# liuzm-slam/VLOAM-NOTED

Measured on AMD Instinct MI355X. Metric: scan-to-map LM iters/sec on 64-ring KITTI-shaped cloud, higher is better.
Workload: dtype fp64 pose/normal equations, fp32 points

## Files before the change

### vloam-noted_amd/csrc/cubeindex.h

```cpp
#pragma once
#include "common.h"
#include "device_math.h"

namespace loam {

constexpr uint32_t CI_EMPTY = 0xFFFFFFFFu;
constexpr uint32_t CI_KEY_MASK = (1u << 18) - 1;
constexpr int CI_LDS_MAX_T = 32768;

__host__ __device__ inline uint32_t ci_table_size(uint32_t n) {
  uint32_t t = 1;
  while (t < 2 * n) t <<= 1;
  return t;
}
__device__ inline uint32_t ci_hash(uint32_t k, uint32_t mask) {
  uint32_t h = k * 0x9E3779B1u;
  h ^= h >> 15;
  return h & mask;
}
__device__ inline int ci_corner(int c, int cen) { return (c - cen) * 50 - 25; }
__device__ inline uint32_t ci_local_key(const float4& p, const int corner[3]) {
  const int lx = (int)floorf(p.x) - corner[0], ly = (int)floorf(p.y) - corner[1], lz = (int)floorf(p.z) - corner[2];
  return (uint32_t)(lx & 63) | ((uint32_t)(ly & 63) << 6) | ((uint32_t)(lz & 63) << 12);
}

template <int nthreads>
__device__ inline uint32_t ci_block_scan(uint32_t v, uint32_t* ws, uint32_t* total) {
  constexpr int W = nthreads / 64;
  const int wid = threadIdx.x >> 6, lane = threadIdx.x & 63;
  const uint32_t inc = wave_incl_scan_u(v);
  if (lane == 63) ws[wid] = inc;
  __syncthreads();
  if (threadIdx.x == 0) {
    uint32_t acc = 0;
    for (int w = 0; w < W; ++w) {
      const uint32_t t = ws[w];
      ws[w] = acc;
      acc += t;
    }
    ws[W] = acc;
  }
  __syncthreads();
  const uint32_t r = ws[wid] + inc - v;
  *total = ws[W];
  __syncthreads();
  return r;
}

template <int nthreads, int MAXT = CI_LDS_MAX_T>
__device__ inline bool cube_index_build(const float4* pts, uint32_t n, const int corner[3], float4* cpts,
                                        uint2* ctab, uint32_t* lds, unsigned long long* prof = nullptr) {
  const int tid = threadIdx.x;
  if (n == 0) return true;
  const uint32_t T = ci_table_size(n), mask = T - 1;
  uint32_t* ws = lds + MAXT;
  bool ok = true;
  if (prof && tid == 0 && T <= (uint32_t)MAXT && n < (1u << 14)) atomicAdd(prof, 0ull - __builtin_readcyclecounter());
  if (T <= (uint32_t)MAXT && n < (1u << 14)) {
    uint32_t* lent = lds;
    for (uint32_t i = tid; i < T; i += nthreads) lent[i] = CI_EMPTY;
    __syncthreads();
    constexpr int PER = (MAXT / 2 + nthreads - 1) / nthreads;
    constexpr int CI_LOADS = PER < 8 ? PER : 8;
    uint32_t sr[PER];
#pragma unroll
    for (int k0 = 0; k0 < PER; k0 += CI_LOADS) {
      float4 p[CI_LOADS];
#pragma unroll
      for (int u = 0; u < CI_LOADS; ++u) p[u] = pts[min(tid + (uint32_t)(k0 + u) * nthreads, n - 1)];
#pragma unroll
      for (int u = 0; u < CI_LOADS; ++u)
        sr[k0 + u] = tid + (uint32_t)(k0 + u) * nthreads < n ? ci_local_key(p[u], corner) : CI_EMPTY;
    }
    const int lane = tid & 63;
    const uint64_t le = lane == 63 ? ~0ull : ((2ull << lane) - 1ull);
#pragma unroll
    for (int k = 0; k < PER; ++k) {
      const uint32_t key = sr[k];
      const uint32_t prev = (uint32_t)__shfl_up((int)key, 1, 64);
      const uint64_t heads = __ballot(lane == 0 || prev != key);
      const int head = 63 - __clzll(heads & le);
      uint32_t base = 0;
      if (key != CI_EMPTY && head == lane) {
        const uint64_t after = heads & ~le;
        const uint32_t run = (uint32_t)((after ? __ffsll((long long)after) - 1 : 64) - lane);
        uint32_t h = ci_hash(key, mask);
        while (true) {
          const uint32_t old = atomicCAS(&lent[h], CI_EMPTY, key | (run << 18));
          if (old == CI_EMPTY) break;
          if ((old & CI_KEY_MASK) == key) {
            base = atomicAdd(&lent[h], run << 18) >> 18;
            break;
          }
          h = (h + 1) & mask;
        }
        base |= h << 15;
      }
      const uint32_t hb = (uint32_t)__shfl((int)base, head, 64);
      sr[k] = key == CI_EMPTY ? CI_EMPTY : hb + (uint32_t)(lane - head);
    }
    __syncthreads();
    if (prof && tid == 0) atomicAdd(prof, __builtin_readcyclecounter());
    uint32_t sum = 0;
    for (uint32_t h = tid; h < T; h += nthreads) {
      const uint32_t e = lent[h];
      if (e != CI_EMPTY) sum += e >> 18;
    }
    uint32_t tot;
    uint32_t pre = ci_block_scan<nthreads>(sum, ws, &tot);
    for (uint32_t h = tid; h < T; h += nthreads) {
      const uint32_t e = lent[h];
      ctab[h] = make_uint2(e, pre);
      lent[h] = pre;
      if (e != CI_EMPTY) pre += e >> 18;
    }
    __syncthreads();
#pragma unroll
    for (int k0 = 0; k0 < PER; k0 += CI_LOADS) {
      float4 p[CI_LOADS];
#pragma unroll
      for (int u = 0; u < CI_LOADS; ++u) p[u] = pts[min(tid + (uint32_t)(k0 + u) * nthreads, n - 1)];
#pragma unroll
      for (int u = 0; u < CI_LOADS; ++u) {
        const uint32_t i = tid + (uint32_t)(k0 + u) * nthreads;
        if (i < n) cpts[lent[sr[k0 + u] >> 15] + (sr[k0 + u] & 0x7FFFu)] = make_float4(p[u].x, p[u].y, p[u].z, __int_as_float((int)i));
      }
    }
    __syncthreads();
    return ok;
  }
  for (uint32_t i = tid; i < T; i += nthreads) ctab[i] = make_uint2(CI_EMPTY, 0);
  __syncthreads();
  for (uint32_t i = tid; i < n; i += nthreads) {
    const uint32_t key = ci_local_key(pts[i], corner);
    uint32_t h = ci_hash(key, mask);
    while (true) {
      const uint32_t old = atomicCAS(&ctab[h].x, CI_EMPTY, key);
      if (old == CI_EMPTY || old == key) break;
      h = (h + 1) & mask;
    }
    atomicAdd(&ctab[h].y, 1u);
  }
  __syncthreads();
  uint32_t sum = 0;
  for (uint32_t h = tid; h < T; h += nthreads) {
    const uint2 e = ctab[h];
    if (e.x != CI_EMPTY) sum += e.y;
  }
  uint32_t tot;
  uint32_t pre = ci_block_scan<nthreads>(sum, ws, &tot);
  for (uint32_t h = tid; h < T; h += nthreads) {
    const uint2 e = ctab[h];
    if (e.x == CI_EMPTY) continue;
    ok &= e.y < (1u << 14);
    ctab[h] = make_uint2(e.x | (e.y << 18), pre);
    pre += e.y;
  }
  __syncthreads();
  for (uint32_t i = tid; i < n; i += nthreads) {
    const float4 p = pts[i];
// ... 29 lines not shown
```

### vloam-noted_amd/csrc/mapper.hip

```cpp
#include <algorithm>
#include <cmath>
#include <cstdlib>
#include <array>
#include <cstring>
#include <deque>
#include <memory>
#include <vector>

#include "common.h"
#include "device_math.h"
#include "cellhash.h"
#include "comm.h"
#include "cubeindex.h"
#include "device_res.h"
#include "lm.h"
#include "voxel.h"
#include "voxel_hot.h"
#include "voxel_pcl.h"
#include "mapper_dev.h"
#include "mapper_stack.h"
#include "mapper_frame.h"
#include "mapper_corr.h"
#include "mapper_lm.h"
#include "mapper_map.h"
// ... 88 lines not shown
  StackIn* sin_buf = nullptr;
  PinnedArray<StackIn> hsin;
};

struct loam_mapper {
  DevStream st;
  DevStream st2;
  int32_t held_rc = 0;
  std::string held_msg;
  loam_params P;
  bool prof = false;
  std::vector<DevEvent> ev_pool;
  std::vector<int> ev_fam;
  double fam_ms[NFAM] = {0}, fam_bytes[NFAM] = {0};
  long long fam_launches[NFAM] = {0};
  int dev = 0, B = 1;
  DevEvent ev_opt_begin, ev_opt_end;
  MapperDev D{};
  PinnedArray<StreamFrame> hf;
  std::vector<HostStream> hs;
  uint2* cube_tab[2] = {nullptr, nullptr};
  int parity = 0;
  uint32_t* tok_tmp = nullptr;
  uint32_t* d_new_off = nullptr;
  DevPool pool;
  uint32_t frame_counter = 0;
  int n_cu = 256;
  uint32_t compact_at = 0;
  int lm_G = 0;
  bool want_ipc = false;
  DevBuf<char> ipc_own;
  std::vector<void*> ipc_open;
  int knn_cs = 0;
  loam_comm* comm = nullptr;
  PinnedArray<int> q_off;
  int* d_q_off = nullptr;
  int use_graph = 0;
  hipGraphExec_t gexec[2][2] = {{nullptr, nullptr}, {nullptr, nullptr}};
  int spar = 0, last_spar = 0;
  ParitySlot slot[2];
  std::deque<FrameRec> q;
  uint64_t seq = 0, mirror_seq = 0;
  unsigned long long stack_seq = 0;
  unsigned long long* d_stk_ready = nullptr;
  PinnedArray<unsigned long long> done;
  unsigned long long* done_dev = nullptr;
// ... 280 lines not shown
  }
  TRY(alloc(D.arena, B * 2 * 2 * (size_t)D.map_cap));
  TRY(alloc(D.carena, B * 2 * 2 * (size_t)D.map_cap));
  TRY(alloc(D.ctab, B * 2 * 2 * 4 * (size_t)D.map_cap));
  TRY(alloc(h->cube_tab[0], B * 2 * NCUBE));
  TRY(alloc(h->cube_tab[1], B * 2 * NCUBE));
  TRY(alloc(D.extra_flag, B * 2 * NCUBE));
  D.knn_stride = B * 2 * (size_t)D.max_in;
  TRY(alloc(D.knn_id, 5 * D.knn_stride));
  TRY(alloc(D.r_type, B * 2 * (size_t)D.max_in));
  TRY(alloc(D.r_px, B * 2 * (size_t)D.max_in));
  TRY(alloc(D.r_py, B * 2 * (size_t)D.max_in));
  TRY(alloc(D.r_pz, B * 2 * (size_t)D.max_in));
  for (int k = 0; k < 3; ++k) {
    TRY(alloc(D.r_a[k], B * 2 * (size_t)D.max_in));
    TRY(alloc(D.r_b[k], B * 2 * (size_t)D.max_in));
  }
  TRY(alloc(D.ins_pts, B * 2 * (size_t)D.max_in));
  TRY(alloc(D.ins_tag, B * 2 * (size_t)D.max_in));
  TRY(alloc(D.ins_sorted, B * 2 * (size_t)D.max_in));
  TRY(alloc(D.ins_off, B * 2 * (size_t)(INS_SLOTS + 1)));
  TRY(alloc(D.stable_tok, B * 2 * (size_t)NCUBE));
  TRY(alloc(h->tok_tmp, B * 2 * (size_t)NCUBE));
  TRY(alloc(D.dbg, LOAM_DEBUG_COUNTERS));
  {
    const char* penv = std::getenv("LOAM_PHASE_COUNTERS");
    D.pdbg = (penv && std::atoi(penv) > 0) ? D.dbg : nullptr;
  }
  TRY(alloc(D.vx_pts, B * 2 * (size_t)D.scratch_cap));
  if (D.pcl_order) {
    const size_t ps = mp_scratch(D);
    TRY(alloc(D.pe, B * 2 * ps));
    TRY(alloc(D.pa, B * 2 * ps));
    TRY(alloc(D.pb, B * 2 * ps));
    TRY(alloc(D.ps, B * 2 * ps));
    TRY(alloc(D.pseg, B * 2 * (mp_pseg(ps) + 9)));
  }
  TRY(alloc(D.vx_idx, B * 2 * (size_t)D.scratch_cap));
  TRY(alloc(D.stk_part, B * 2 * (size_t)STACK_K_MAX));
  for (ParitySlot& S : h->slot) {
    TRY(alloc(S.stk_n_buf, B * 2));
    TRY(alloc(S.stk_err_buf, B));
    if (B <= 4) {
      TRY(S.hsin.assign_mapped(B, StackIn{}, &S.sin_buf));
    } else {
      TRY(alloc(S.sin_buf, B));
// ... 90 lines not shown
  do {                                                                                      \
    if ((h) && !(h)->q.empty() && !(h)->q.front().behind && !(h)->q.front().early_seen) { \
      LOAM_HIP(hipSetDevice((h)->dev));                                                     \
      TRY(finish_oldest(h));                                                                \
    }                                                                                       \
  } while (0)

int32_t loam_mapper_destroy(loam_mapper* h) {
  if (!h) return LOAM_ERR_ARG;
  (void)hipSetDevice(h->dev);
  while (!h->q.empty()) (void)finish_oldest(h);
  delete h;
  return LOAM_OK;
}

int32_t loam_mapper_reset(loam_mapper* h) {
  if (!h) return LOAM_ERR_ARG;
  SETTLE(h);
  LOAM_HIP(hipSetDevice(h->dev));
  LOAM_HIP(hipStreamSynchronize(h->st2));
  for (int p = 0; p < 2; ++p)
    LOAM_HIP(hipMemsetAsync(h->cube_tab[p], 0, sizeof(uint2) * h->B * 2 * NCUBE, h->st));
  LOAM_HIP(hipMemsetAsync(h->D.stable_tok, 0, sizeof(uint32_t) * h->B * 2 * NCUBE, h->st));
  LOAM_HIP(hipStreamSynchronize(h->st));
  for (int s = 0; s < h->B; ++s) {
    h->hf[s] = fresh_record();
    h->last_tail[s] = {0u, 0u};
    h->hs[s] = HostStream{};
  }
  return LOAM_OK;
}

static int32_t mapper_input_common(loam_mapper* h, int32_t s, const float* corner, int32_t nc,
                                   const float* surf, int32_t ns, const double* q_wodom,
                                   const double* t_wodom, int32_t skip, hipMemcpyKind kind) {
  TRY(check_stream(h, s));
  if (!q_wodom || !t_wodom || nc < 0 || ns < 0 || (nc > 0 && !corner) || (ns > 0 && !surf)) {
    set_error("loam_mapper_input: bad arguments");
    return LOAM_ERR_ARG;
  }
  if (nc > h->D.max_in || ns > h->D.max_in) {
    set_error("loam_mapper_input: cloud larger than max_input_points");
    return LOAM_ERR_CAPACITY;
  }
  LOAM_HIP(hipSetDevice(h->dev));
  HostStream& H = h->hs[s];
// ... 288 lines not shown
      capture_frame(h, D, fpar, st);
      LOAM_HIP(hipStreamEndCapture(st, &gr));
      const hipError_t ie = hipGraphInstantiate(&ge, gr, nullptr, nullptr, 0);
      (void)hipGraphDestroy(gr);
      LOAM_HIP(ie);
    }
    if (!chained) LOAM_HIP(hipMemcpyAsync(D.fr, h->hf.data(), sizeof(StreamFrame) * B, hipMemcpyHostToDevice, st));
    if (compact_due) TRY(launch_compaction(h, D, due_at, st));
    if (!chained) LOAM_HIP(hipEventRecord(S.ev_fr[0], st));
    if (direct) {
      capture_frame(h, D, fpar, st);
      LOAM_HIP(hipGetLastError());
    } else {
      LOAM_HIP(hipGraphLaunch(ge, st));
    }
    if (!chained) LOAM_HIP(hipEventRecord(S.ev_fr[1], st));
    return LOAM_OK;
  }
  LOAM_HIP(hipMemcpyAsync(D.fr, h->hf.data(), sizeof(StreamFrame) * B, hipMemcpyHostToDevice, st));
  LOAM_HIP(hipEventRecord(S.ev_fr[0], st));
  if (compact_due) TRY(launch_compaction(h, D, due_at, st));
  if (any_shift) {
    LAUNCH(FAM_OTHER, k_shift_cubes<<<dim3(16, B), 256, 0, st>>>(D, h->cube_tab[h->parity],
                                                                 h->cube_tab[1 - h->parity], h->tok_tmp));
    LOAM_HIP(hipMemcpyAsync(D.stable_tok, h->tok_tmp, sizeof(uint32_t) * B * 2 * NCUBE, hipMemcpyDeviceToDevice, st));
    h->parity ^= 1;
    D.cube_tab = h->cube_tab[h->parity];
  }
  const bool multi = D.sharded && D.nrank > 1;
  if (D.sharded) {
    LAUNCH(FAM_OTHER, k_submap_count<<<B, 256, 0, st>>>(D));
    if (multi) TRY(comm_allreduce(h->comm, D.wcnt, (int64_t)B * 2 * WIN_MAX, LOAM_DT_I32, st));
  }
  LAUNCH(FAM_OTHER, k_submap_prep<<<B, 128, 0, st>>>(D));
  LOAM_HIP(hipEventRecord(h->ev_opt_begin, st));
  LOAM_HIP(hipStreamWaitEvent(st, h->ev_stack, 0));
  LAUNCH(FAM_OTHER, k_stack_counts<<<B, 64, 0, st>>>(D));
  size_t q_tot = 0;
  if (multi) {
    int* qo = h->q_off.data() + (size_t)fpar * (B + 1);
    for (int s = 0; s < B; ++s) {
      const StreamFrame& F = h->hf[s];
      qo[s] = (int)q_tot;
      if (F.active) q_tot += (size_t)F.nc_in + F.ns_in;
    }
    qo[B] = (int)q_tot;
    LOAM_HIP(hipMemcpyAsync(h->d_q_off, qo, sizeof(int) * (B + 1), hipMemcpyHostToDevice, st));
  }
// ... 363 lines not shown
        }
    h->early = true;
  }
  TRY(loam_mapper_solve_async(h));
  while (h->q.size() > 1) TRY(finish_oldest_held(h));
  TRY(launch_front(h));
  if (h->q.empty()) return take_held(h);
  FrameRec& R = h->q.front();
  bool early = R.graph && !R.pending;
  if (early) TRY(wait_word(h, h->done_early.data() + R.fpar, R.epoch));
  if (!early || !take_early(h, R)) {
    const int32_t rc = finish_oldest(h);
    if (rc != LOAM_OK) return rc;
  }
  return take_held(h);
}

int32_t loam_mapper_debug_counters(loam_mapper* h, uint64_t* out, int32_t n, int32_t reset) {
  SETTLE(h);
  if (!h || !out || n < 0 || n > LOAM_DEBUG_COUNTERS) return LOAM_ERR_ARG;
  LOAM_HIP(hipSetDevice(h->dev));
  LOAM_HIP(hipStreamSynchronize(h->st));
  LOAM_HIP(hipMemcpy(out, h->D.dbg, sizeof(uint64_t) * n, hipMemcpyDeviceToHost));
  if (reset) LOAM_HIP(hipMemset(h->D.dbg, 0, sizeof(uint64_t) * LOAM_DEBUG_COUNTERS));
  return LOAM_OK;
}

int32_t loam_mapper_set_profiling(loam_mapper* h, int32_t enable) {
  SETTLE(h);
  if (!h) return LOAM_ERR_ARG;
  h->prof = enable != 0;
  h->ev_fam.clear();
  return LOAM_OK;
}

int32_t loam_mapper_kernel_times(loam_mapper* h, loam_kernel_times* out) {
  SETTLE(h);
  if (!h || !out) return LOAM_ERR_ARG;
  for (int f = 0; f < LOAM_KFAM_COUNT; ++f) {
    out->ms[f] = f < NFAM ? h->fam_ms[f] : 0.0;
    out->launches[f] = f < NFAM ? h->fam_launches[f] : 0;
    out->bytes[f] = f < NFAM ? h->fam_bytes[f] : 0.0;
  }
  return LOAM_OK;
}

// ... 216 lines not shown
```

### vloam-noted_amd/csrc/mapper_corr.h

```cpp
#pragma once

namespace loam {

struct Near5 {
  float d[5];
  int id[5];
  int pos[5];
};
__device__ inline void near5_offer(Near5& T, float d, int id, int pos) {
  if (!(d < T.d[4] || (d == T.d[4] && id < T.id[4]))) return;
  T.d[4] = d; T.id[4] = id; T.pos[4] = pos;
#pragma unroll
  for (int k = 4; k > 0; --k) {
    if (T.d[k] < T.d[k - 1] || (T.d[k] == T.d[k - 1] && T.id[k] < T.id[k - 1])) {
      float td = T.d[k]; T.d[k] = T.d[k - 1]; T.d[k - 1] = td;
      int ti = T.id[k]; T.id[k] = T.id[k - 1]; T.id[k - 1] = ti;
      int tp = T.pos[k]; T.pos[k] = T.pos[k - 1]; T.pos[k - 1] = tp;
    }
  }
}
__device__ inline int floor_div50(int v) { return v >= 0 ? v / 50 : -((-v + 49) / 50); }

struct WinMap {
  uint32_t off[WIN_MAX], n[WIN_MAX], tsize[WIN_MAX];
  int sub[WIN_MAX];
};

__device__ inline void corr_block(const MapperDev& D, int* s, int* blk) {
  *s = D.s0 + blockIdx.x % D.B;
  *blk = blockIdx.x / D.B;
}

#ifndef KNN_WAVES
#define KNN_WAVES 7
#endif
template <int L, bool CS = false>
__global__ void __launch_bounds__(CORR_THREADS) __attribute__((amdgpu_waves_per_eu(CS ? 4 : KNN_WAVES, 8))) k_knn(MapperDev D, int round) {
  __shared__ WinMap W[2];
  __shared__ int slot_of[75];
  int s, blk;
  corr_block(D, &s, &blk);
  StreamFrame& F = D.fr[s];
  if (!F.active) return;
  double X[7];
#pragma unroll
  for (int i = 0; i < 7; ++i) X[i] = F.pose[i];
  if (blk == 0 && threadIdx.x < LM_SYNC_WORDS) D.lm_sync[((size_t)s * 2 + round) * LM_SYNC_WORDS + threadIdx.x] = 0;
  if (blk == 0 && threadIdx.x == 0) {
    lm_init(F.lm[round], X, 4, F.optimize != 0);
#pragma unroll
    for (int i = 0; i < 7; ++i) F.knn_pose[i] = X[i];
  }
  if (!F.optimize) return;
  const int tid = threadIdx.x;
  const int c0 = F.center[0] - 2, c1 = F.center[1] - 2, c2 = F.center[2] - 1;
  if (tid < 75) slot_of[tid] = -1;
  __syncthreads();
  if (tid < F.valid_num) {
    const int cube = F.window[tid];
    const int ci = cube % CW, cj = (cube / CW) % CH, ck = cube / (CW * CH);
    slot_of[(ci - c0) * 15 + (cj - c1) * 3 + (ck - c2)] = tid;
#pragma unroll
    for (int m = 0; m < 2; ++m) {
      const uint2 cv = D.cube_tab[sm_index(s, m) * NCUBE + cube];
      W[m].off[tid] = cv.x;
      W[m].n[tid] = cv.y;
      W[m].tsize[tid] = cv.y ? ci_table_size(cv.y) : 0u;
      W[m].sub[tid] = F.sub_off[m][tid];
    }
  }
  __syncthreads();
  const int nc = F.nc_stack, ns = F.ns_stack;
  const size_t rb = (size_t)s * 2 * D.max_in;
  uint32_t ncand = 0;
  const int gsub = tid % L;
  const int nblk = CS ? D.knn_blk : CORR_BLK;
  for (int ridx = blk * (CORR_THREADS / L) + tid / L; ridx < nc + ns; ridx += nblk * (CORR_THREADS / L)) {
    const int m = ridx < nc ? 0 : 1;
    const int qi = m == 0 ? ridx : ridx - nc;
    const float4 q = to_map(X, D.stack[m][(size_t)s * D.max_in + qi]);
    const float4* cp = carena_base(D, s, m, F.arena_active[m]);
    const uint2* ct = ctab_base(D, s, m, F.arena_active[m]);
    const WinMap& WM = W[m];
    Near5 T;
#pragma unroll
    for (int k = 0; k < 5; ++k) {
      T.d[k] = INFINITY;
// ... 4 lines not shown
    const int qx = (int)fx, qy = (int)fy, qz = (int)fz;
    const float lx = q.x - fx, hx = (fx + 1.0f) - q.x;
    const float ly = q.y - fy, hy = (fy + 1.0f) - q.y;
    const float lz = q.z - fz, hz = (fz + 1.0f) - q.z;
    auto scan = [&](int bi, int bj, int bk, int ax, int ay, int az) {
      const int wx = bi - c0, wy = bj - c1, wz = bk - c2;
      if (wx < 0 || wx > 4 || wy < 0 || wy > 4 || wz < 0 || wz > 2) return;
      const int sl = slot_of[wx * 15 + wy * 3 + wz];
      if (sl < 0) return;
      const uint32_t n = WM.n[sl];
      if (n == 0) return;
      const uint32_t off = WM.off[sl];
      const uint2 e = ci_find(ct + 4 * (size_t)off, WM.tsize[sl],
                              (uint32_t)ax | ((uint32_t)ay << 6) | ((uint32_t)az << 12));
      ncand += e.y;
      const int sub = WM.sub[sl];
      for (uint32_t k = CS ? 0 : gsub; k < e.y; k += CS ? 1 : L) {
        const uint32_t pos = off + e.x + k;
        const float4 p = cp[pos];
        const int key = (sub + __float_as_int(p.w)) * D.nrank + D.rank;
        near5_offer(T, fdist2(q.x, q.y, q.z, p.x, p.y, p.z), key, (int)pos);
      }
    };
    for (int ob = 0; ob < 27; ob += CS ? L : 1) {
      const int o = CS ? ob + gsub : ob;
      const uint32_t code = cell_order_code(o < 27 ? o : 0);
      const int dx = (int)(code & 3u) - 1, dy = (int)((code >> 2) & 3u) - 1, dz = (int)(code >> 4) - 1;
      const float gx = dx < 0 ? lx : (dx > 0 ? hx : 0.f);
      const float gy = dy < 0 ? ly : (dy > 0 ? hy : 0.f);
      const float gz = dz < 0 ? lz : (dz > 0 ? hz : 0.f);
      float bound = fminf(T.d[4], 1.0f) * 1.01f + 1e-6f;
#pragma unroll
      for (int o2 = 1; o2 < L; o2 <<= 1) bound = fminf(bound, __shfl_xor(bound, o2, 64));
      if (o >= 27 || gx * gx + gy * gy + gz * gz > bound) continue;
      const int x = qx + dx, y = qy + dy, z = qz + dz;
      const int bi = floor_div50(x + 25) + F.cen[0], bj = floor_div50(y + 25) + F.cen[1],
                bk = floor_div50(z + 25) + F.cen[2];
      int cx[3] = {bi, bj, bk};
      int lc[3];
      const int cv[3] = {x, y, z};
#pragma unroll
      for (int a = 0; a < 3; ++a) lc[a] = cv[a] - ci_corner(cx[a], F.cen[a]);
      scan(bi, bj, bk, lc[0], lc[1], lc[2]);
      int edge = 0;
#pragma unroll
      for (int a = 0; a < 3; ++a)
        if (cv[a] + 25 < 0 && (cv[a] + 25) % 50 == 0) edge |= 1 << a;
      for (int e = edge; e; e = (e - 1) & edge) {
        int b2[3], l2[3];
#pragma unroll
        for (int a = 0; a < 3; ++a) {
          b2[a] = (e >> a) & 1 ? cx[a] - 1 : cx[a];
          l2[a] = (e >> a) & 1 ? 50 : lc[a];
        }
        scan(b2[0], b2[1], b2[2], l2[0], l2[1], l2[2]);
      }
    }
#pragma unroll
    for (int o = 1; o < L; o <<= 1) {
      float pd[5];
      int pid[5], ppos[5];
#pragma unroll
      for (int k = 0; k < 5; ++k) {
        pd[k] = __shfl_xor(T.d[k], o, 64);
        pid[k] = __shfl_xor(T.id[k], o, 64);
        ppos[k] = __shfl_xor(T.pos[k], o, 64);
      }
#pragma unroll
      for (int k = 0; k < 5; ++k)
        if (ppos[k] >= 0) near5_offer(T, pd[k], pid[k], ppos[k]);
    }
    if (gsub != 0) continue;
    if (D.sharded) {
      NnRec& o = D.nn_send[D.q_off[s] + ridx];
#pragma unroll
      for (int k = 0; k < 5; ++k) {
        o.d[k] = T.d[k];
        o.id[k] = T.id[k];
// ... 169 lines not shown
```

### vloam-noted_amd/csrc/mapper_dev.h

```cpp
#pragma once

namespace loam {

constexpr int CW = 21, CH = 21, CD = 11, NCUBE = CW * CH * CD;
constexpr int WIN_MAX = 125;
constexpr int WIN_VALID_MAX = 75;
constexpr int EXTRA_CAP = 64;
constexpr int CORR_THREADS = 128;
constexpr int CORR_BLK = 128;
static_assert(CORR_THREADS >= WIN_VALID_MAX, "k_knn window tables");
constexpr int LM_THREADS = 256;
constexpr int LM_EBLK = 32;
constexpr int INS_SLOTS = WIN_VALID_MAX + EXTRA_CAP;
constexpr int RQ_CLASSES = 8;
constexpr int MAP_ERR_SUBMAP = 4, MAP_ERR_EXTRA = 8, MAP_ERR_HASH = 16, MAP_ERR_LM_SYNC = 32,
              MAP_ERR_INDEX = 64, MAP_ERR_LIVE = 128, MAP_ERR_SORT = 256,
              MAP_ERR_STACK = 512, MAP_ERR_STACK_WAIT = 2048;

enum MapDbg {
  MD_REVOX_CYC = 0 , MD_MERGE_NEW_PTS = 3, MD_REVOX_ITEMS = 4 , MD_MERGES = 7,
  MD_INDEX_CYC = 8, MD_INDEX_PTS = 9, MD_OLD_PTS = 10, MD_CUBE_SEG = 11 , MD_INDEX_HASH_CYC = 16,
  MD_LM = 17 , MD_REVOX_SIZE_ITEMS = 24 , MD_REVOX_SIZE_CYC = 32 ,
  MD_POSE_DIFF = 40, MD_COMPACTIONS = 41, MD_STACK_SEG = 42 , MD_COMPACTIONS_MAP = 48 ,
  MD_CUBE_HOT = 50, MD_STACK_HOT = 54, MD_PREP_CYC = 58 ,
  MD_PREP_LAUNCHES = 62, MD_PREP_ON_DEVICE = 63, MD_CUBE_GLOB = 64, MD_STACK_GLOB = 65, MD_CUBE_HEAP = 66 ,
  MD_STACK_HEAP = 68 , MD_CUBE_SORT = 72, MD_STACK_SORT = 77, MD_CUBE_WAVES = 82, MD_STACK_CUTS = 91,
  MD_DBG_END = 92
};
static_assert(MD_POSE_DIFF == 40 && MD_COMPACTIONS == 41 && MD_COMPACTIONS_MAP + 1 == 49, "slots the tests read by number");
static_assert(MD_CUBE_HOT + VHF_SLOTS <= MD_STACK_HOT && MD_STACK_HOT + VHF_SLOTS <= MD_PREP_CYC &&
                  MD_CUBE_SORT + VHS_SLOTS == MD_STACK_SORT && MD_STACK_SORT + VHS_SLOTS == MD_CUBE_WAVES &&
                  MD_CUBE_WAVES + VHD_SLOTS == MD_STACK_CUTS && MD_CUBE_SEG + VXM_SLOTS <= MD_INDEX_HASH_CYC &&
                  MD_STACK_SEG + VXS_SLOTS == MD_COMPACTIONS_MAP && MD_DBG_END <= LOAM_DEBUG_COUNTERS,
              "counter slots");

struct StreamFrame {
  double pose[7];
  int active;
  uint32_t epoch;
  int nc_in, ns_in;
  int nc_stack, ns_stack;
  int sub_n[2];
  int optimize;
  int corner_num[2], surf_num[2];
  int valid_num;
  int window[WIN_MAX];
  int sub_off[2][WIN_MAX + 1];
  int center[3];
  int cen[3];
  int shift[3];
  int origin[3];
// ... 30 lines not shown
  int n[2];
  int active;
  int pad;
};

struct MapPose {
  double x[7];
};

struct MapperDev {
  int B;
  int s0 = 0;
  int max_in, map_cap, sub_cap, scratch_cap, max_chunks;
  float leaf[2];
  uint32_t epoch;
  StreamFrame* fr;
  float4* in_pts[2];
  float4* stack[2];
  float4* arena;
  float4* carena;
  uint2* ctab;
  uint2* cube_tab;
  uint32_t* extra_flag;
  int* knn_id;
  size_t knn_stride;
  int* r_type;
  float* r_px;
  float* r_py;
  float* r_pz;
  double* r_a[3];
  double* r_b[3];
  float4* ins_pts;
  int* ins_tag;
  float4* ins_sorted;
  uint32_t* ins_off;
  unsigned long long* dbg;
  unsigned long long* pdbg;
  uint32_t* stable_tok;
  float4* vx_pts;
  int* vx_idx;
  double* partials;
  uint32_t* lm_sync;
  double* lm_xpub;
  uint32_t* tickets;
  uint32_t* lm_tick;
  uint32_t* rq;
// ... 36 lines not shown
struct NnRec {
  float d[5];
  int id[5];
  float x[5], y[5], z[5];
};

__device__ inline size_t sm_index(int s, int m) { return (size_t)s * 2 + m; }

__device__ inline float4* arena_base(const MapperDev& D, int s, int m, int active) {
  return D.arena + ((sm_index(s, m) * 2 + active) * (size_t)D.map_cap);
}
__device__ inline float4* carena_base(const MapperDev& D, int s, int m, int active) {
  return D.carena + ((sm_index(s, m) * 2 + active) * (size_t)D.map_cap);
}
__device__ inline uint2* ctab_base(const MapperDev& D, int s, int m, int active) {
  return D.ctab + ((sm_index(s, m) * 2 + active) * (size_t)D.map_cap * 4);
}
__device__ inline void cube_corner(int c, const int* cen, int corner[3]) {
  corner[0] = ci_corner(c % CW, cen[0]);
  corner[1] = ci_corner((c / CW) % CH, cen[1]);
  corner[2] = ci_corner(c / (CW * CH), cen[2]);
}

__global__ void k_shift_cubes(MapperDev D, const uint2* __restrict__ old_tab, uint2* new_tab, uint32_t* tok_tmp) {
  int s = D.s0 + blockIdx.y;
  const StreamFrame& F = D.fr[s];
  for (int t = blockIdx.x * blockDim.x + threadIdx.x; t < 2 * NCUBE; t += gridDim.x * blockDim.x) {
    int m = t / NCUBE, c = t % NCUBE;
    int i = c % CW, j = (c / CW) % CH, k = c / (CW * CH);
    int oi = i - F.shift[0], oj = j - F.shift[1], ok = k - F.shift[2];
    uint2 v = make_uint2(0, 0);
    uint32_t tok = 0;
    if (oi >= 0 && oi < CW && oj >= 0 && oj < CH && ok >= 0 && ok < CD) {
      const size_t o = sm_index(s, m) * NCUBE + oi + CW * oj + CW * CH * ok;
      v = old_tab[o];
      tok = D.stable_tok[o];
    }
    new_tab[sm_index(s, m) * NCUBE + c] = v;
    tok_tmp[sm_index(s, m) * NCUBE + c] = tok;
  }
}

}
```

### vloam-noted_amd/csrc/mapper_map.h

```cpp
#pragma once

namespace loam {

__device__ inline bool revox_target(const MapperDev& D, int s, int m, int slot, int* cube_out, int* append_out) {
  const StreamFrame& F = D.fr[s];
  if (!F.active) return false;
  int cube, append;
  if (slot < F.valid_num) {
    cube = F.window[slot];
    append = 0;
  } else if (slot >= WIN_VALID_MAX && slot - WIN_VALID_MAX < min(F.extra_n[m], EXTRA_CAP)) {
    cube = F.extra_list[m][slot - WIN_VALID_MAX];
    append = 1;
  } else {
    return false;
  }
  const uint32_t* ioff = D.ins_off + sm_index(s, m) * (INS_SLOTS + 1);
  const uint32_t n_new = ioff[slot + 1] - ioff[slot];
  const uint2 cv = D.cube_tab[sm_index(s, m) * NCUBE + cube];
  if (!append && n_new == 0 && (cv.y == 0 || D.stable_tok[sm_index(s, m) * NCUBE + cube] == cv.x + 1))
    return false;
  *cube_out = cube;
  *append_out = append;
  return true;
// ... 150 lines not shown
  static_assert(INS_SLOTS <= VX_THREADS, "one thread per slot");
  if (my_cube >= 0) {
    const bool append = tid >= WIN_VALID_MAX;
    if (append || my_new != 0 || (my_cv.y != 0 && my_tok != my_cv.x + 1)) {
      const uint32_t nt = my_cv.y + my_new;
      const int c = nt < 1024u ? 0 : min(RQ_CLASSES - 1, 32 - __clz(nt >> 10));
      const uint32_t k = atomicAdd(&D.rq_ctl[c], 1u);
      D.rq[(size_t)c * D.rq_cap + k] = (uint32_t)(sm * INS_SLOTS + tid);
    }
  }
}

#ifndef REVOX_PROF_MIN_N
#define REVOX_PROF_MIN_N 0
#endif
template <bool PCL>
__device__ inline void revox_item(MapperDev& D, int s, int m, int slot, int cube, int append, uint32_t* lds) {
  StreamFrame& F = D.fr[s];
  const uint32_t* ioff = D.ins_off + sm_index(s, m) * (INS_SLOTS + 1);
  const uint32_t i0 = ioff[slot], n_new = ioff[slot + 1] - i0;
  uint32_t* tok = D.stable_tok + sm_index(s, m) * NCUBE + cube;
  uint2* tab = D.cube_tab + sm_index(s, m) * NCUBE;
  const uint2 cv = tab[cube];
  if (cv.y + n_new < (uint32_t)REVOX_PROF_MIN_N) D.pdbg = nullptr;
  float4* ar = arena_base(D, s, m, F.arena_active[m]);
  VoxSeg S;
  S.src0 = ar + cv.x;
  S.n0 = (int)cv.y;
  S.src1 = D.ins_sorted + sm_index(s, m) * D.max_in + i0;
  S.tag1 = nullptr;
  S.n1 = (int)n_new;
  S.tag = cube;
  S.leaf = D.leaf[m];
  S.append_only = append;
  S.out = ar;
  S.tail = &F.arena_tail[m];
  S.cap = D.map_cap;
  S.res_off = &tab[cube].x;
  S.res_cnt = &tab[cube].y;
  S.stable_out = tok;
  S.scratch_pts = D.vx_pts + sm_index(s, m) * D.scratch_cap;
  S.scratch_idx = D.vx_idx + sm_index(s, m) * D.scratch_cap;
  S.scratch_tail = &F.scratch_tail[m];
  S.scratch_cap = D.scratch_cap;
  S.err = &F.err;
  S.prof = D.pdbg ? D.pdbg + MD_CUBE_SEG : nullptr;
// ... 1 lines not shown
  cube_corner(cube, F.cen, S.anchor);
  bool merged = false;
  const unsigned long long t0 = __builtin_readcyclecounter();
  const bool fixed = n_new > 0 && n_new <= VX_MERGE_CAP && cv.y > 0 && *tok == cv.x + 1;
  if (PCL && !append) {
    uint32_t* sb = vx_park_block(lds);
    if (threadIdx.x == 0) *sb = atomicAdd(&F.hot_tail[m], cv.y + n_new + MP_SLACK);
    __syncthreads();
    const uint32_t so = *sb;
    __syncthreads();
    S.hot = map_hot(D, sm_index(s, m), so, cv.y + n_new);
    map_filter_exact(D, sm_index(s, m), so, S, VxSrc{S.src0, S.n0, S.src1}, lds, &tab[cube], fixed, &merged);
    __syncthreads();
  } else {
    if (!append && fixed) {
      merged = vx_merge_fixed_point(S, lds);
      __syncthreads();
    }
    if (!merged) voxel_segment(S, lds);
    __syncthreads();
  }
  const unsigned long long t1 = __builtin_readcyclecounter();
  uint32_t* res = vx_park_result(lds);
  if (threadIdx.x == 0) {
    const uint2 v = tab[cube];
    res[0] = v.x;
    res[1] = v.y;
  }
  __syncthreads();
  const uint32_t off = res[0], n = res[1];
  __syncthreads();
  int corner[3];
  cube_corner(cube, F.cen, corner);
  if (!cube_index_build<VX_THREADS, CI_LDS_MAX_T>(ar + off, n, corner, carena_base(D, s, m, F.arena_active[m]) + off,
                                  ctab_base(D, s, m, F.arena_active[m]) + 4 * (size_t)off, lds, D.pdbg ? D.pdbg + MD_INDEX_HASH_CYC : nullptr) &&
      threadIdx.x == 0)
    atomicOr(&F.err, MAP_ERR_INDEX);
  if (threadIdx.x == 0)
    atomicAdd(&F.vx_bytes, 16ull * (cv.y + n_new) + 16ull * 3 * n + (n ? 8ull * ci_table_size(n) : 0ull));
  if (threadIdx.x == 0 && D.pdbg) {
    const unsigned long long t2 = __builtin_readcyclecounter();
    const int k = merged ? 0 : (append ? 2 : 1);
    atomicAdd(&D.dbg[MD_REVOX_CYC + k], t1 - t0);
    atomicAdd(&D.dbg[MD_REVOX_ITEMS + k], 1ull);
    atomicAdd(&D.dbg[MD_INDEX_CYC], t2 - t1);
    atomicAdd(&D.dbg[MD_INDEX_PTS], (unsigned long long)n);
    atomicAdd(&D.dbg[MD_OLD_PTS], (unsigned long long)cv.y);
    int hb = 0;
    while (hb < 7 && n >= (1024u << hb)) ++hb;
    atomicAdd(&D.dbg[MD_REVOX_SIZE_ITEMS + hb], 1ull);
    atomicAdd(&D.dbg[MD_REVOX_SIZE_CYC + hb], t2 - t0);
    if (merged) {
      atomicAdd(&D.dbg[MD_MERGE_NEW_PTS], (unsigned long long)n_new);
      atomicAdd(&D.dbg[MD_MERGES], 1ull);
    }
  }
}

template <bool PCL>
__global__ void __launch_bounds__(VX_THREADS) k_revox(MapperDev D) {
  __shared__ __attribute__((aligned(16))) uint32_t lds[VX_LDS_WORDS];
  uint32_t b = blockIdx.x;
  int item = -1;
  for (int c = RQ_CLASSES - 1; c >= 0; --c) {
    const uint32_t nc = D.rq_ctl[c];
    if (b < nc) {
      item = (int)D.rq[(size_t)c * D.rq_cap + b];
      break;
    }
    b -= nc;
  }
  if (item < 0) return;
  const int slot = item % INS_SLOTS, sm = item / INS_SLOTS;
  int cube = 0, append = 0;
  if (!revox_target(D, sm >> 1, sm & 1, slot, &cube, &append)) return;
  revox_item<PCL>(D, sm >> 1, sm & 1, slot, cube, append, lds);
}

__global__ void __launch_bounds__(VX_THREADS) k_cube_index(MapperDev D, int s, int m, int c0, int c1,
                                                           int3 cen) {
  __shared__ __attribute__((aligned(16))) uint32_t lds[CI_LDS_MAX_T + VX_WAVES + 1];
  const int cube = c0 + blockIdx.x;
  if (cube >= c1) return;
  StreamFrame& F = D.fr[s];
  const uint2 cv = D.cube_tab[sm_index(s, m) * NCUBE + cube];
  if (cv.y == 0) return;
  const int cenv[3] = {cen.x, cen.y, cen.z};
  int corner[3];
  cube_corner(cube, cenv, corner);
  const int active = F.arena_active[m];
  if (!cube_index_build<VX_THREADS>(arena_base(D, s, m, active) + cv.x, cv.y, corner,
                                    carena_base(D, s, m, active) + cv.x,
                                    ctab_base(D, s, m, active) + 4 * (size_t)cv.x, lds) &&
      threadIdx.x == 0)
    atomicOr(&F.err, MAP_ERR_INDEX);
}

__device__ inline bool compact_due(const MapperDev& D, int sm) {
  return D.fr[sm >> 1].arena_tail[sm & 1] > D.compact_due_at;
}

__global__ void k_compact_scan(MapperDev D, uint32_t* new_off) {
  __shared__ uint32_t ws[VX_WAVES + 1];
  const int sm = 2 * D.s0 + blockIdx.x;
  if (!compact_due(D, sm)) return;
  const uint2* tab = D.cube_tab + (size_t)sm * NCUBE;
  uint32_t* no = new_off + (size_t)blockIdx.x * (NCUBE + 1);
  constexpr int PER = (NCUBE + VX_THREADS - 1) / VX_THREADS;
  uint32_t v[PER];
  uint32_t sum = 0;
#pragma unroll
  for (int k = 0; k < PER; ++k) {
    int c = threadIdx.x * PER + k;
    v[k] = c < NCUBE ? tab[c].y : 0u;
    sum += v[k];
  }
// ... 102 lines not shown
```

Before: 548,800.

## Add per-cube voxel occupancy bitmaps to skip empty KNN neighbour cells

While building each cube's hash index, the change also builds a 51x51x51 occupancy bitmap per cube in LDS and writes it to a pooled global buffer. Blocks come from a bitmask allocator and are released when cubes leave the window during shifts. The non-cooperative KNN path then reads the nine relevant bitmap rows up front to form a 27-bit mask of occupied neighbour cells, and visits only those cells instead of hashing into all 27. This costs more LDS and global writes during index builds, adds allocator and shift bookkeeping, and risks stale or incorrect bitmaps, which would make the search miss neighbours.

Measured after the change: 589,100, median of 6. +7.4%, better.

```diff
diff --git a/vloam-noted_amd/csrc/cubeindex.h b/vloam-noted_amd/csrc/cubeindex.h
--- a/vloam-noted_amd/csrc/cubeindex.h
+++ b/vloam-noted_amd/csrc/cubeindex.h
@@ -7,6 +7,10 @@
 constexpr uint32_t CI_EMPTY = 0xFFFFFFFFu;
 constexpr uint32_t CI_KEY_MASK = (1u << 18) - 1;
 constexpr int CI_LDS_MAX_T = 32768;
+constexpr int CI_OCC_DIM = 51;
+constexpr int CI_OCC_WORDS = 2602;
+constexpr int CI_OCC_LDS = 2 * CI_OCC_WORDS;
+constexpr int CI_OCC_LDS_AT = 32;
 
 __host__ __device__ inline uint32_t ci_table_size(uint32_t n) {
   uint32_t t = 1;
@@ -47,18 +51,30 @@
   return r;
 }
 
+__device__ inline bool ci_occ_bit(uint32_t key, uint32_t* word, uint32_t* bit) {
+  const uint32_t lx = key & 63u, ly = (key >> 6) & 63u, lz = (key >> 12) & 63u;
+  *word = 2u * (lz * CI_OCC_DIM + ly) + (lx >> 5);
+  *bit = 1u << (lx & 31u);
+  return lx < (uint32_t)CI_OCC_DIM && ly < (uint32_t)CI_OCC_DIM && lz < (uint32_t)CI_OCC_DIM;
+}
+
 template <int nthreads, int MAXT = CI_LDS_MAX_T>
 __device__ inline bool cube_index_build(const float4* pts, uint32_t n, const int corner[3], float4* cpts,
-                                        uint2* ctab, uint32_t* lds, unsigned long long* prof = nullptr) {
+                                        uint2* ctab, uint32_t* lds, unsigned long long* prof = nullptr,
+                                        uint64_t* occ = nullptr, bool occ_fresh = true) {
+  static_assert(nthreads / 64 + 1 <= CI_OCC_LDS_AT && (MAXT + CI_OCC_LDS_AT) % 4 == 0, "block image after the scan words");
   const int tid = threadIdx.x;
   if (n == 0) return true;
   const uint32_t T = ci_table_size(n), mask = T - 1;
   uint32_t* ws = lds + MAXT;
+  uint32_t* locc = lds + MAXT + CI_OCC_LDS_AT;
   bool ok = true;
   if (prof && tid == 0 && T <= (uint32_t)MAXT && n < (1u << 14)) atomicAdd(prof, 0ull - __builtin_readcyclecounter());
   if (T <= (uint32_t)MAXT && n < (1u << 14)) {
     uint32_t* lent = lds;
     for (uint32_t i = tid; i < T; i += nthreads) lent[i] = CI_EMPTY;
+    if (occ)
+      for (uint32_t i = tid; i < (uint32_t)CI_OCC_LDS; i += nthreads) locc[i] = 0u;
     __syncthreads();
     constexpr int PER = (MAXT / 2 + nthreads - 1) / nthreads;
     constexpr int CI_LOADS = PER < 8 ? PER : 8;
@@ -87,7 +103,11 @@
         uint32_t h = ci_hash(key, mask);
         while (true) {
           const uint32_t old = atomicCAS(&lent[h], CI_EMPTY, key | (run << 18));
-          if (old == CI_EMPTY) break;
+          if (old == CI_EMPTY) {
+            uint32_t ow, ob;
+            if (occ && ci_occ_bit(key, &ow, &ob)) atomicOr(&locc[ow], ob);
+            break;
+          }
           if ((old & CI_KEY_MASK) == key) {
             base = atomicAdd(&lent[h], run << 18) >> 18;
             break;
@@ -101,6 +121,14 @@
     }
     __syncthreads();
     if (prof && tid == 0) atomicAdd(prof, __builtin_readcyclecounter());
+    if (occ) {
+      const uint4* src = reinterpret_cast<const uint4*>(locc);
+      uint4* dst = reinterpret_cast<uint4*>(occ);
+      for (uint32_t i = tid; i < (uint32_t)CI_OCC_LDS / 4; i += nthreads) {
+        const uint4 v = src[i];
+        if (occ_fresh || (v.x | v.y | v.z | v.w)) dst[i] = v;
+      }
+    }
     uint32_t sum = 0;
     for (uint32_t h = tid; h < T; h += nthreads) {
       const uint32_t e = lent[h];
@@ -130,12 +158,18 @@
     return ok;
   }
   for (uint32_t i = tid; i < T; i += nthreads) ctab[i] = make_uint2(CI_EMPTY, 0);
+  if (occ && occ_fresh)
+    for (uint32_t i = tid; i < (uint32_t)CI_OCC_WORDS; i += nthreads) occ[i] = 0ull;
   __syncthreads();
   for (uint32_t i = tid; i < n; i += nthreads) {
     const uint32_t key = ci_local_key(pts[i], corner);
     uint32_t h = ci_hash(key, mask);
     while (true) {
       const uint32_t old = atomicCAS(&ctab[h].x, CI_EMPTY, key);
+      if (old == CI_EMPTY) {
+        uint32_t ow, ob;
+        if (occ && ci_occ_bit(key, &ow, &ob)) atomicOr(reinterpret_cast<uint32_t*>(occ) + ow, ob);
+      }
       if (old == CI_EMPTY || old == key) break;
       h = (h + 1) & mask;
     }
diff --git a/vloam-noted_amd/csrc/mapper.hip b/vloam-noted_amd/csrc/mapper.hip
--- a/vloam-noted_amd/csrc/mapper.hip
+++ b/vloam-noted_amd/csrc/mapper.hip
@@ -134,6 +134,7 @@
   uint2* cube_tab[2] = {nullptr, nullptr};
   int parity = 0;
   uint32_t* tok_tmp = nullptr;
+  uint32_t* occ_tmp = nullptr;
   uint32_t* d_new_off = nullptr;
   DevPool pool;
   uint32_t frame_counter = 0;
@@ -460,6 +461,16 @@
   TRY(alloc(D.ins_off, B * 2 * (size_t)(INS_SLOTS + 1)));
   TRY(alloc(D.stable_tok, B * 2 * (size_t)NCUBE));
   TRY(alloc(h->tok_tmp, B * 2 * (size_t)NCUBE));
+  {
+    const char* oenv = std::getenv("LOAM_KNN_OCC");
+    const char* benv = std::getenv("LOAM_KNN_OCC_BLOCKS");
+    D.occ_blocks = (h->knn_cs || (oenv && oenv[0] == '0')) ? 0 : OCC_POOL;
+    if (D.occ_blocks && benv) D.occ_blocks = std::max(1, std::min(OCC_POOL, std::atoi(benv)));
+    TRY(alloc(D.cube_occ, B * 2 * (size_t)NCUBE));
+    TRY(alloc(h->occ_tmp, B * 2 * (size_t)NCUBE));
+    TRY(alloc(D.occ_used, B * 2 * (size_t)OCC_USED_WORDS));
+    TRY(alloc(D.occ_pool, B * 2 * (size_t)D.occ_blocks * CI_OCC_WORDS));
+  }
   TRY(alloc(D.dbg, LOAM_DEBUG_COUNTERS));
   {
     const char* penv = std::getenv("LOAM_PHASE_COUNTERS");
@@ -596,6 +607,8 @@
   for (int p = 0; p < 2; ++p)
     LOAM_HIP(hipMemsetAsync(h->cube_tab[p], 0, sizeof(uint2) * h->B * 2 * NCUBE, h->st));
   LOAM_HIP(hipMemsetAsync(h->D.stable_tok, 0, sizeof(uint32_t) * h->B * 2 * NCUBE, h->st));
+  LOAM_HIP(hipMemsetAsync(h->D.cube_occ, 0, sizeof(uint32_t) * h->B * 2 * NCUBE, h->st));
+  LOAM_HIP(hipMemsetAsync(h->D.occ_used, 0, sizeof(uint32_t) * h->B * 2 * OCC_USED_WORDS, h->st));
   LOAM_HIP(hipStreamSynchronize(h->st));
   for (int s = 0; s < h->B; ++s) {
     h->hf[s] = fresh_record();
@@ -930,8 +943,9 @@
   if (compact_due) TRY(launch_compaction(h, D, due_at, st));
   if (any_shift) {
     LAUNCH(FAM_OTHER, k_shift_cubes<<<dim3(16, B), 256, 0, st>>>(D, h->cube_tab[h->parity],
-                                                                 h->cube_tab[1 - h->parity], h->tok_tmp));
+                                                                 h->cube_tab[1 - h->parity], h->tok_tmp, h->occ_tmp));
     LOAM_HIP(hipMemcpyAsync(D.stable_tok, h->tok_tmp, sizeof(uint32_t) * B * 2 * NCUBE, hipMemcpyDeviceToDevice, st));
+    LOAM_HIP(hipMemcpyAsync(D.cube_occ, h->occ_tmp, sizeof(uint32_t) * B * 2 * NCUBE, hipMemcpyDeviceToDevice, st));
     h->parity ^= 1;
     D.cube_tab = h->cube_tab[h->parity];
   }
@@ -1341,6 +1355,12 @@
   LOAM_HIP(hipSetDevice(h->dev));
   LOAM_HIP(hipStreamSynchronize(h->st));
   LOAM_HIP(hipMemcpy(out, h->D.dbg, sizeof(uint64_t) * n, hipMemcpyDeviceToHost));
+  if (n > MD_OCC_IN_USE) {
+    std::vector<uint32_t> used((size_t)h->B * 2 * OCC_USED_WORDS);
+    LOAM_HIP(hipMemcpy(used.data(), h->D.occ_used, sizeof(uint32_t) * used.size(), hipMemcpyDeviceToHost));
+    out[MD_OCC_IN_USE] = 0;
+    for (uint32_t w : used) out[MD_OCC_IN_USE] += (uint64_t)__builtin_popcount(w);
+  }
   if (reset) LOAM_HIP(hipMemset(h->D.dbg, 0, sizeof(uint64_t) * LOAM_DEBUG_COUNTERS));
   return LOAM_OK;
 }
diff --git a/vloam-noted_amd/csrc/mapper_corr.h b/vloam-noted_amd/csrc/mapper_corr.h
--- a/vloam-noted_amd/csrc/mapper_corr.h
+++ b/vloam-noted_amd/csrc/mapper_corr.h
@@ -38,6 +38,7 @@
 __global__ void __launch_bounds__(CORR_THREADS) __attribute__((amdgpu_waves_per_eu(CS ? 4 : KNN_WAVES, 8))) k_knn(MapperDev D, int round) {
   __shared__ WinMap W[2];
   __shared__ int slot_of[75];
+  __shared__ uint32_t wocc[2][75];
   int s, blk;
   corr_block(D, &s, &blk);
   StreamFrame& F = D.fr[s];
@@ -55,6 +56,7 @@
   const int tid = threadIdx.x;
   const int c0 = F.center[0] - 2, c1 = F.center[1] - 2, c2 = F.center[2] - 1;
   if (tid < 75) slot_of[tid] = -1;
+  if (L == 1 && !CS && tid < 75) wocc[0][tid] = wocc[1][tid] = OCC_ABSENT;
   __syncthreads();
   if (tid < F.valid_num) {
     const int cube = F.window[tid];
@@ -63,6 +65,7 @@
 #pragma unroll
     for (int m = 0; m < 2; ++m) {
       const uint2 cv = D.cube_tab[sm_index(s, m) * NCUBE + cube];
+      if (L == 1 && !CS && cv.y) wocc[m][(ci - c0) * 15 + (cj - c1) * 3 + (ck - c2)] = D.cube_occ[sm_index(s, m) * NCUBE + cube];
       W[m].off[tid] = cv.x;
       W[m].n[tid] = cv.y;
       W[m].tsize[tid] = cv.y ? ci_table_size(cv.y) : 0u;
@@ -113,17 +116,7 @@
         near5_offer(T, fdist2(q.x, q.y, q.z, p.x, p.y, p.z), key, (int)pos);
       }
     };
-    for (int ob = 0; ob < 27; ob += CS ? L : 1) {
-      const int o = CS ? ob + gsub : ob;
-      const uint32_t code = cell_order_code(o < 27 ? o : 0);
-      const int dx = (int)(code & 3u) - 1, dy = (int)((code >> 2) & 3u) - 1, dz = (int)(code >> 4) - 1;
-      const float gx = dx < 0 ? lx : (dx > 0 ? hx : 0.f);
-      const float gy = dy < 0 ? ly : (dy > 0 ? hy : 0.f);
-      const float gz = dz < 0 ? lz : (dz > 0 ? hz : 0.f);
-      float bound = fminf(T.d[4], 1.0f) * 1.01f + 1e-6f;
-#pragma unroll
-      for (int o2 = 1; o2 < L; o2 <<= 1) bound = fminf(bound, __shfl_xor(bound, o2, 64));
-      if (o >= 27 || gx * gx + gy * gy + gz * gz > bound) continue;
+    auto visit = [&](int dx, int dy, int dz) {
       const int x = qx + dx, y = qy + dy, z = qz + dz;
       const int bi = floor_div50(x + 25) + F.cen[0], bj = floor_div50(y + 25) + F.cen[1],
                 bk = floor_div50(z + 25) + F.cen[2];
@@ -145,6 +138,103 @@
           l2[a] = (e >> a) & 1 ? 50 : lc[a];
         }
         scan(b2[0], b2[1], b2[2], l2[0], l2[1], l2[2]);
+      }
+    };
+    if constexpr (L == 1 && !CS) {
+      uint32_t cells = 0x7FFFFFFu;
+      if (D.occ_blocks) {
+        const uint64_t* pool = D.occ_pool + sm_index(s, m) * D.occ_blocks * (size_t)CI_OCC_WORDS;
+        const uint32_t* wo = wocc[m];
+        const int qv[3] = {qx, qy, qz};
+        int wb[3][3], lo[3][3];
+        uint32_t open[3] = {0u, 0u, 0u};
+#pragma unroll
+        for (int a = 0; a < 3; ++a) {
+#pragma unroll
+          for (int d = 0; d < 3; ++d) {
+            const int v = qv[a] + d - 1;
+            const int bc = floor_div50(v + 25) + F.cen[a];
+            wb[a][d] = bc - (a == 0 ? c0 : (a == 1 ? c1 : c2));
+            lo[a][d] = v - ci_corner(bc, F.cen[a]);
+            if (v + 25 < 0 && (v + 25) % 50 == 0) open[a] |= 1u << d;
+          }
+        }
+        if (wb[0][0] != wb[0][1]) open[0] |= 1u;
+        if (wb[0][2] != wb[0][1]) open[0] |= 4u;
+        uint64_t row[9];
+#pragma unroll
+        for (int r = 0; r < 9; ++r) {
+          const int dy = r % 3, dz = r / 3;
+          const int wx = wb[0][1], wy = wb[1][dy], wz = wb[2][dz];
+          const bool in = wx >= 0 && wx <= 4 && wy >= 0 && wy <= 4 && wz >= 0 && wz <= 2;
+          const uint32_t id = in ? wo[wx * 15 + wy * 3 + wz] : OCC_ABSENT;
+          const bool has = id != OCC_ABSENT && id != OCC_NONE;
+          const uint64_t w = pool[has ? (size_t)(id - 1) * CI_OCC_WORDS + (size_t)(lo[2][dz] * CI_OCC_DIM + lo[1][dy]) : 0];
+          row[r] = has ? w : (id == OCC_ABSENT ? 0ull : ~0ull);
+          if ((open[1] >> dy | open[2] >> dz) & 1u) row[r] = ~0ull;
+        }
+        const int sh = lo[0][1] > 0 ? lo[0][1] - 1 : 0;
+        const int up = lo[0][1] > 0 ? 0 : 1;
+        cells = 0u;
+#pragma unroll
+        for (int o = 0; o < 27; ++o) {
+          const uint32_t code = cell_order_code(o);
+          const int dx = (int)(code & 3u), dy = (int)((code >> 2) & 3u), dz = (int)(code >> 4);
+          const uint32_t t3 = ((uint32_t)(row[dz * 3 + dy] >> sh) << up) | open[0];
+          cells |= ((t3 >> dx) & 1u) << o;
+        }
+      }
+      while (true) {
+        const float bound = fminf(T.d[4], 1.0f) * 1.01f + 1e-6f;
+        int dx = 0, dy = 0, dz = 0;
+        bool found = false;
+        while (cells && !found) {
+          const int o = __builtin_ctz(cells);
+          cells &= cells - 1u;
+          const uint32_t code = cell_order_code(o);
+          dx = (int)(code & 3u) - 1, dy = (int)((code >> 2) & 3u) - 1, dz = (int)(code >> 4) - 1;
+          const float gx = dx < 0 ? lx : (dx > 0 ? hx : 0.f);
+          const float gy = dy < 0 ? ly : (dy > 0 ? hy : 0.f);
+          const float gz = dz < 0 ? lz : (dz > 0 ? hz : 0.f);
+          found = !(gx * gx + gy * gy + gz * gz > bound);
+        }
+        if (!found) break;
+        visit(dx, dy, dz);
+      }
+    } else {
+      for (int ob = 0; ob < 27; ob += CS ? L : 1) {
+        const int o = CS ? ob + gsub : ob;
+        const uint32_t code = cell_order_code(o < 27 ? o : 0);
+        const int dx = (int)(code & 3u) - 1, dy = (int)((code >> 2) & 3u) - 1, dz = (int)(code >> 4) - 1;
+        const float gx = dx < 0 ? lx : (dx > 0 ? hx : 0.f);
+        const float gy = dy < 0 ? ly : (dy > 0 ? hy : 0.f);
+        const float gz = dz < 0 ? lz : (dz > 0 ? hz : 0.f);
+        float bound = fminf(T.d[4], 1.0f) * 1.01f + 1e-6f;
+#pragma unroll
+        for (int o2 = 1; o2 < L; o2 <<= 1) bound = fminf(bound, __shfl_xor(bound, o2, 64));
+        if (o >= 27 || gx * gx + gy * gy + gz * gz > bound) continue;
+        const int x = qx + dx, y = qy + dy, z = qz + dz;
+        const int bi = floor_div50(x + 25) + F.cen[0], bj = floor_div50(y + 25) + F.cen[1],
+                  bk = floor_div50(z + 25) + F.cen[2];
+        int cx[3] = {bi, bj, bk};
+        int lc[3];
+        const int cv[3] = {x, y, z};
+  #pragma unroll
+        for (int a = 0; a < 3; ++a) lc[a] = cv[a] - ci_corner(cx[a], F.cen[a]);
+        scan(bi, bj, bk, lc[0], lc[1], lc[2]);
+        int edge = 0;
+  #pragma unroll
+        for (int a = 0; a < 3; ++a)
+          if (cv[a] + 25 < 0 && (cv[a] + 25) % 50 == 0) edge |= 1 << a;
+        for (int e = edge; e; e = (e - 1) & edge) {
+          int b2[3], l2[3];
+  #pragma unroll
+          for (int a = 0; a < 3; ++a) {
+            b2[a] = (e >> a) & 1 ? cx[a] - 1 : cx[a];
+            l2[a] = (e >> a) & 1 ? 50 : lc[a];
+          }
+          scan(b2[0], b2[1], b2[2], l2[0], l2[1], l2[2]);
+        }
       }
     }
 #pragma unroll
diff --git a/vloam-noted_amd/csrc/mapper_dev.h b/vloam-noted_amd/csrc/mapper_dev.h
--- a/vloam-noted_amd/csrc/mapper_dev.h
+++ b/vloam-noted_amd/csrc/mapper_dev.h
@@ -25,8 +25,12 @@
   MD_CUBE_HOT = 50, MD_STACK_HOT = 54, MD_PREP_CYC = 58 ,
   MD_PREP_LAUNCHES = 62, MD_PREP_ON_DEVICE = 63, MD_CUBE_GLOB = 64, MD_STACK_GLOB = 65, MD_CUBE_HEAP = 66 ,
   MD_STACK_HEAP = 68 , MD_CUBE_SORT = 72, MD_STACK_SORT = 77, MD_CUBE_WAVES = 82, MD_STACK_CUTS = 91,
-  MD_DBG_END = 92
-};
+  MD_OCC_IN_USE = 92 , MD_OCC_ALLOC_FAIL = 93,
+  MD_DBG_END = 94
+};
+constexpr int OCC_POOL = 160, OCC_USED_WORDS = OCC_POOL / 32;
+static_assert(OCC_POOL >= WIN_MAX && OCC_POOL % 32 == 0, "occupancy pool");
+constexpr uint32_t OCC_ABSENT = 0xFFFFFFFFu, OCC_NONE = 0u;
 static_assert(MD_POSE_DIFF == 40 && MD_COMPACTIONS == 41 && MD_COMPACTIONS_MAP + 1 == 49, "slots the tests read by number");
 static_assert(MD_CUBE_HOT + VHF_SLOTS <= MD_STACK_HOT && MD_STACK_HOT + VHF_SLOTS <= MD_PREP_CYC &&
                   MD_CUBE_SORT + VHS_SLOTS == MD_STACK_SORT && MD_STACK_SORT + VHS_SLOTS == MD_CUBE_WAVES &&
@@ -103,6 +107,10 @@
   uint2* ctab;
   uint2* cube_tab;
   uint32_t* extra_flag;
+  uint32_t* cube_occ;
+  uint32_t* occ_used;
+  uint64_t* occ_pool;
+  int occ_blocks = 0;
   int* knn_id;
   size_t knn_stride;
   int* r_type;
@@ -185,7 +193,47 @@
   corner[2] = ci_corner(c / (CW * CH), cen[2]);
 }
 
-__global__ void k_shift_cubes(MapperDev D, const uint2* __restrict__ old_tab, uint2* new_tab, uint32_t* tok_tmp) {
+__device__ inline uint64_t* occ_block(const MapperDev& D, size_t sm, uint32_t id) {
+  return D.occ_pool + (sm * D.occ_blocks + (id - 1)) * (size_t)CI_OCC_WORDS;
+}
+__device__ inline void occ_release(const MapperDev& D, size_t sm, uint32_t id) {
+  atomicAnd(&D.occ_used[sm * OCC_USED_WORDS + (id - 1) / 32], ~(1u << ((id - 1) & 31)));
+}
+__device__ inline uint32_t occ_alloc(const MapperDev& D, size_t sm) {
+  uint32_t* used = D.occ_used + sm * OCC_USED_WORDS;
+  for (int w = 0; 32 * w < D.occ_blocks; ++w) {
+    const int nb = D.occ_blocks - 32 * w;
+    const uint32_t valid = nb >= 32 ? 0xFFFFFFFFu : (1u << nb) - 1u;
+    uint32_t cur = atomicOr(&used[w], 0u);
+    while (~cur & valid) {
+      const int b = __ffs((int)(~cur & valid)) - 1;
+      cur = atomicOr(&used[w], 1u << b);
+      if (!((cur >> b) & 1u)) return (uint32_t)(32 * w + b + 1);
+    }
+  }
+  return 0;
+}
+constexpr uint32_t OCC_FRESH = 0x80000000u;
+__device__ inline uint32_t occ_acquire(const MapperDev& D, size_t sm, int cube, uint32_t n) {
+  if (!D.occ_blocks) return 0;
+  uint32_t* slot = D.cube_occ + sm * NCUBE + cube;
+  uint32_t id = *slot;
+  if (n == 0) {
+    if (id) {
+      occ_release(D, sm, id);
+      *slot = 0;
+    }
+    return 0;
+  }
+  if (id) return id;
+  id = occ_alloc(D, sm);
+  if (id) *slot = id;
+  else atomicAdd(&D.dbg[MD_OCC_ALLOC_FAIL], 1ull);
+  return id ? id | OCC_FRESH : 0u;
+}
+
+__global__ void k_shift_cubes(MapperDev D, const uint2* __restrict__ old_tab, uint2* new_tab, uint32_t* tok_tmp,
+                              uint32_t* occ_tmp) {
   int s = D.s0 + blockIdx.y;
   const StreamFrame& F = D.fr[s];
   for (int t = blockIdx.x * blockDim.x + threadIdx.x; t < 2 * NCUBE; t += gridDim.x * blockDim.x) {
@@ -193,14 +241,19 @@
     int i = c % CW, j = (c / CW) % CH, k = c / (CW * CH);
     int oi = i - F.shift[0], oj = j - F.shift[1], ok = k - F.shift[2];
     uint2 v = make_uint2(0, 0);
-    uint32_t tok = 0;
+    uint32_t tok = 0, occ = 0;
     if (oi >= 0 && oi < CW && oj >= 0 && oj < CH && ok >= 0 && ok < CD) {
       const size_t o = sm_index(s, m) * NCUBE + oi + CW * oj + CW * CH * ok;
       v = old_tab[o];
       tok = D.stable_tok[o];
+      occ = D.cube_occ[o];
     }
     new_tab[sm_index(s, m) * NCUBE + c] = v;
     tok_tmp[sm_index(s, m) * NCUBE + c] = tok;
+    occ_tmp[sm_index(s, m) * NCUBE + c] = occ;
+    const int ni = i + F.shift[0], nj = j + F.shift[1], nk = k + F.shift[2];
+    const uint32_t mine = D.cube_occ[sm_index(s, m) * NCUBE + c];
+    if (mine && (ni < 0 || ni >= CW || nj < 0 || nj >= CH || nk < 0 || nk >= CD)) occ_release(D, sm_index(s, m), mine);
   }
 }
 
diff --git a/vloam-noted_amd/csrc/mapper_map.h b/vloam-noted_amd/csrc/mapper_map.h
--- a/vloam-noted_amd/csrc/mapper_map.h
+++ b/vloam-noted_amd/csrc/mapper_map.h
@@ -196,6 +196,7 @@
   uint32_t* tok = D.stable_tok + sm_index(s, m) * NCUBE + cube;
   uint2* tab = D.cube_tab + sm_index(s, m) * NCUBE;
   const uint2 cv = tab[cube];
+  const uint32_t occ0 = D.occ_blocks ? D.cube_occ[sm_index(s, m) * NCUBE + cube] : 0u;
   if (cv.y + n_new < (uint32_t)REVOX_PROF_MIN_N) D.pdbg = nullptr;
   float4* ar = arena_base(D, s, m, F.arena_active[m]);
   VoxSeg S;
@@ -243,18 +244,21 @@
   }
   const unsigned long long t1 = __builtin_readcyclecounter();
   uint32_t* res = vx_park_result(lds);
+  uint32_t* occ_id = vx_park_block(lds);
   if (threadIdx.x == 0) {
     const uint2 v = tab[cube];
     res[0] = v.x;
     res[1] = v.y;
-  }
-  __syncthreads();
-  const uint32_t off = res[0], n = res[1];
+    *occ_id = (occ0 && v.y) ? occ0 : occ_acquire(D, sm_index(s, m), cube, v.y);
+  }
+  __syncthreads();
+  const uint32_t off = res[0], n = res[1], oid = *occ_id;
   __syncthreads();
   int corner[3];
   cube_corner(cube, F.cen, corner);
   if (!cube_index_build<VX_THREADS, CI_LDS_MAX_T>(ar + off, n, corner, carena_base(D, s, m, F.arena_active[m]) + off,
-                                  ctab_base(D, s, m, F.arena_active[m]) + 4 * (size_t)off, lds, D.pdbg ? D.pdbg + MD_INDEX_HASH_CYC : nullptr) &&
+                                  ctab_base(D, s, m, F.arena_active[m]) + 4 * (size_t)off, lds, D.pdbg ? D.pdbg + MD_INDEX_HASH_CYC : nullptr,
+                                  oid ? occ_block(D, sm_index(s, m), oid & ~OCC_FRESH) : nullptr, (oid & OCC_FRESH) != 0) &&
       threadIdx.x == 0)
     atomicOr(&F.err, MAP_ERR_INDEX);
   if (threadIdx.x == 0)
@@ -278,6 +282,7 @@
   }
 }
 
+static_assert(CI_LDS_MAX_T + CI_OCC_LDS_AT + CI_OCC_LDS <= VX_LDS_WORDS - VX_TAIL_WORDS, "index build LDS");
 template <bool PCL>
 __global__ void __launch_bounds__(VX_THREADS) k_revox(MapperDev D) {
   __shared__ __attribute__((aligned(16))) uint32_t lds[VX_LDS_WORDS];
@@ -300,11 +305,14 @@
 
 __global__ void __launch_bounds__(VX_THREADS) k_cube_index(MapperDev D, int s, int m, int c0, int c1,
                                                            int3 cen) {
-  __shared__ __attribute__((aligned(16))) uint32_t lds[CI_LDS_MAX_T + VX_WAVES + 1];
+  __shared__ __attribute__((aligned(16))) uint32_t lds[CI_LDS_MAX_T + CI_OCC_LDS_AT + CI_OCC_LDS];
+  __shared__ uint32_t occ_id;
   const int cube = c0 + blockIdx.x;
   if (cube >= c1) return;
   StreamFrame& F = D.fr[s];
   const uint2 cv = D.cube_tab[sm_index(s, m) * NCUBE + cube];
+  if (threadIdx.x == 0) occ_id = occ_acquire(D, sm_index(s, m), cube, cv.y);
+  __syncthreads();
   if (cv.y == 0) return;
   const int cenv[3] = {cen.x, cen.y, cen.z};
   int corner[3];
@@ -312,7 +320,8 @@
   const int active = F.arena_active[m];
   if (!cube_index_build<VX_THREADS>(arena_base(D, s, m, active) + cv.x, cv.y, corner,
                                     carena_base(D, s, m, active) + cv.x,
-                                    ctab_base(D, s, m, active) + 4 * (size_t)cv.x, lds) &&
+                                    ctab_base(D, s, m, active) + 4 * (size_t)cv.x, lds, nullptr,
+                                    occ_id ? occ_block(D, sm_index(s, m), occ_id & ~OCC_FRESH) : nullptr, (occ_id & OCC_FRESH) != 0) &&
       threadIdx.x == 0)
     atomicOr(&F.err, MAP_ERR_INDEX);
 }
```
